# CVPR23/Depth-guided-Texture-Diffusion-for-Image-Semantic-Segmentation

Hardware: AMD Instinct MI355X
Metric: training images/sec (512x512 RGB-D, bs=8 per GPU; fwd+loss+bwd+allreduce+AdamW) (higher is better)
Workload: dtype bf16; 1 GPU; config/sod.yml model `cod` (pvt_v2_b2 + ConvNeXt-B texture diffuser + Hitnet decoder), 512x512 RGB+depth, batch 8/GPU, random init, DropPath active; mode=train, global_batch=8, parallelism=dp1, hip_graph=True, graph_mode=single

## Files before the change

### depth-guided-texture-diffusion-for-image-semantic-segmentation_amd/_lib.py

```python
from __future__ import annotations

import ctypes as C
import os

import torch

_HERE = os.path.dirname(os.path.abspath(__file__))
LIB_PATH = os.path.join(_HERE, "libdgtd.so")

F32, BF16, F64, F16 = 0, 1, 2, 3
_vp, _fp, _i, _i64, _f = C.c_void_p, C.c_void_p, C.c_int, C.c_int64, C.c_float

SIGNATURES = {
    "dgtd_version": (_i, []),
    "dgtd_last_error": (C.c_char_p, []),
    "dgtd_profile_enable": (_i, [_i]),
    "dgtd_profile_dump": (_i64, [C.c_char_p, _i64]),
    "dgtd_profile_empty": (_i, [_vp]),
    "dgtd_gemm_supported": (_i, [_i, _i, _i, _i]),
    "dgtd_gemm_bias": (_i, [_vp, _vp, _vp, _vp, _i, _i, _i, _i, _vp]),
    "dgtd_gemm_bias_gelu": (_i, [_vp, _vp, _vp, _vp, _vp, _i, _i, _i, _i, _vp]),
    "dgtd_gemm_bias_residual": (_i, [_vp, _vp, _vp, _vp, _fp, _fp, _vp, _vp, _i, _i, _i, _i64, _i, _vp]),
    "dgtd_gemm_gelu_bwd_workspace": (_i64, [_i, _i]),
    "dgtd_gemm_gelu_bwd": (_i, [_vp, _vp, _vp, _vp, _vp, C.POINTER(C.c_int), _i, _i, _i, _i, _vp]),
# ... 5 lines not shown
    "dgtd_layernorm_bwd_workspace": (_i64, [_i]),
    "dgtd_layernorm_bwd": (_i, [_vp, _vp, _fp, _fp, _fp, _vp, _fp, _fp, _vp, _i64, _i, _i, _vp]),
    "dgtd_layernorm_bwd_partial": (_i, [_vp, _vp, _fp, _fp, _fp, _vp, _vp, _vp, _i64, _i, _i, C.POINTER(C.c_int), _vp]),
    "dgtd_multi_reduce": (_i, [_vp, _i, _vp]),
    "dgtd_scale_residual_bias_bwd_partial": (_i, [_vp, _vp, _fp, _fp, _vp, _vp, _i64, _i, _i64, _i, C.POINTER(C.c_int), _vp]),
    "dgtd_gelu_bias_bwd_partial": (_i, [_vp, _vp, _vp, _vp, _i64, _i, _i, C.POINTER(C.c_int), _vp]),
    "dgtd_colsum_partial": (_i, [_vp, _vp, _i64, _i, _i, C.POINTER(C.c_int), _vp]),
    "dgtd_layernorm_bwd_add": (_i, [_vp, _vp, _fp, _fp, _fp, _vp, _vp, _fp, _fp, _vp, _i64, _i, _i, _vp]),
    "dgtd_sra_attn_fwd": (_i, [_vp, _vp, _vp, _fp, _i, _i, _i, _i, _f, _i, _vp]),
    "dgtd_sra_attn_bwd_workspace": (_i64, [_i, _i, _i]),
    "dgtd_sra_attn_bwd": (_i, [_vp, _vp, _vp, _vp, _fp, _vp, _fp, _vp, _i, _i, _i, _i, _f, _i, _vp]),
    "dgtd_dwconv_fwd": (_i, [_vp, _fp, _fp, _vp, _vp, _i, _i, _i, _i, _i, _i, _i, _vp]),
    "dgtd_dwconv_bwd_weight_workspace": (_i64, [_i, _i, _i, _i, _i]),
    "dgtd_dwconv_bwd_weight": (_i, [_vp, _vp, _fp, _i, _vp, _i, _i, _i, _i, _i, _i, _vp]),
    "dgtd_dwconv_bwd_weight_partial": (_i, [_vp, _vp, _i, _vp, _i, _i, _i, _i, _i, _i, C.POINTER(C.c_int), _vp]),
    "dgtd_dwconv_bwd_weight_batched_blocks": (_i, [_i, _i, _i, _i, _i, _i]),
    "dgtd_dwconv_bwd_weight_batched": (_i, [_vp, _vp, _i, _i, _vp, _i, _i, _i, _i, _i, _i, _vp]),
    "dgtd_dwconv_pack_batched": (_i, [_vp, _vp, _vp, _vp, _vp, _i, _i, _vp]),
    "dgtd_dwconv_pack": (_i, [_vp, _vp, _fp, _i, _i, _i, _vp]),
    "dgtd_dwconv_unpack_grads": (_i, [_fp, _vp, _vp, _i, _i, _i, _vp]),
    "dgtd_scale_residual_fwd": (_i, [_vp, _vp, _fp, _fp, _vp, _i64, _i, _i64, _i, _vp]),
    "dgtd_colsum_workspace": (_i64, [_i]),
    "dgtd_scale_residual_bwd": (_i, [_vp, _vp, _fp, _fp, _vp, _fp, _vp, _i64, _i, _i64, _i, _vp]),
    "dgtd_colsum": (_i, [_vp, _vp, _i, _vp, _i64, _i, _i, _vp]),
    "dgtd_colsum2_workspace": (_i64, [_i]),
    "dgtd_scale_residual_bias_bwd": (_i, [_vp, _vp, _fp, _fp, _vp, _fp, _vp, _i, _vp, _i64, _i, _i64, _i, _vp]),
    "dgtd_gelu_bias_bwd": (_i, [_vp, _vp, _vp, _vp, _i, _vp, _i64, _i, _i, _vp]),
    "dgtd_seg_loss_workspace": (_i64, [_i, _i]),
    "dgtd_seg_loss_fwd": (_i, [_fp, _fp, _fp, _fp, _vp, _i, _i, _i, _vp]),
    "dgtd_seg_loss_bwd": (_i, [_fp, _fp, _fp, _fp, _fp, _vp, _i, _i, _i, _vp]),
    "dgtd_ssim_workspace": (_i64, []),
    "dgtd_ssim_value": (_i, [_fp, _fp, _fp, _vp, _i, _i, _i, _vp]),
    "dgtd_diffuser_fwd": (_i, [_fp, _fp, _fp, _fp, _fp, _fp, _fp, _i, _i, _vp]),
    "dgtd_diffuser_bwd": (_i, [_fp, _fp, _fp, _fp, _fp, _fp, _fp, _fp, _fp, _fp, _fp, _i, _i, _vp]),
    "dgtd_diffuse_tail_fwd": (_i, [_fp, _fp, _fp, _fp, _fp, _i, _i, _vp]),
    "dgtd_diffuse_tail_bwd_workspace": (_i64, [_i]),
    "dgtd_diffuse_tail_bwd": (_i, [_fp, _fp, _fp, _fp, _fp, _fp, _vp, _i, _i, _vp]),
    "dgtd_adamw_flat": (_i, [_fp, _fp, _fp, _fp, _vp, _i64, _f, _f, _f, _f, _f, _f, _f, _vp]),
    "dgtd_adamw_flat_amp": (_i, [_fp, _fp, _fp, _fp, _vp, _i, _i64, _f, _f, _f, _f, _f, _f, _f, _fp, _fp, _vp]),
    "dgtd_adamw_flat_g16": (_i, [_fp, _vp, _fp, _fp, _vp, _i, _i64, _f, _f, _f, _f, _f, _f, _f, _fp, _fp, _vp]),
    "dgtd_adamw_flat_clip": (_i, [_fp, _fp, _vp, _fp, _fp, _vp, _i, _i64, _f, _f, _f, _f, _f, _f, _f, _fp, _fp, _fp, _f, _vp]),
    "dgtd_grad_norm_partial": (_i, [_vp, _i, _i64, _i, _vp, _i, _vp]),
    "dgtd_grad_clip_finalize": (_i, [_vp, _i64, _i, _f, _fp, _fp, _vp]),
    "dgtd_found_inf": (_i, [_fp, _i64, _fp, _vp]),
    "dgtd_loss_scale_update": (_i, [_fp, _f, _f, _i, _vp]),
    "dgtd_im2col": (_i, [_vp, _vp, _i, _i, _i, _i, _i64, _i64, _i64, _i64, _i, _i, _i, _i, _i, _i, _i, _vp]),
# ... 127 lines not shown
```

### depth-guided-texture-diffusion-for-image-semantic-segmentation_amd/csrc/elementwise.hip

```cpp
#include "common.h"

namespace {

constexpr int EW_MAX_BLOCKS = 512;

template <typename T>
__global__ __launch_bounds__(256) void scale_residual_fwd_kernel(const T* __restrict__ x, const T* __restrict__ y,
                                                                 const float* __restrict__ s, const float* __restrict__ gamma,
                                                                 T* __restrict__ out, int64_t rows, int C, int64_t rows_per_sample) {
  typedef typename Vec16<T>::type VT;
  constexpr int V = Vec16<T>::N;
  const int CV = C / V;
  const int64_t total = rows * CV;
  for (int64_t i = (int64_t)blockIdx.x * 256 + threadIdx.x; i < total; i += (int64_t)gridDim.x * 256) {
    const int cv = (int)(i % CV);
    const int64_t r = i / CV;
    const float sb = s ? s[r / rows_per_sample] : 1.f;
    VT xv = *reinterpret_cast<const VT*>(x + i * V);
    VT yv = *reinterpret_cast<const VT*>(y + i * V);
    VT o;
#pragma unroll
    for (int j = 0; j < V; ++j) {
      const float g = gamma ? gamma[cv * V + j] : 1.f;
      o[j] = (T)((float)xv[j] + sb * g * (float)yv[j]);
    }
    *reinterpret_cast<VT*>(out + i * V) = o;
  }
}

template <typename T, int MODE>
__global__ __launch_bounds__(256) void colsum_kernel(const T* __restrict__ g, const T* __restrict__ y, const float* __restrict__ s,
                                                     const float* __restrict__ gamma, T* __restrict__ dy, float* __restrict__ ws,
                                                     int64_t rows, int C, int64_t rows_per_sample) {
  typedef typename Vec16<T>::type VT;
  constexpr int V = Vec16<T>::N;
  extern __shared__ float red[];
  const int CV = C / V;
  const int CVB = min(CV - (int)blockIdx.y * 256, 256);
  const int RG = 256 / CVB;
  const int tid = threadIdx.x;
  const int cvl = tid % CVB, rg = tid / CVB;
  const int cv = blockIdx.y * 256 + cvl;
  float acc[V];
#pragma unroll
  for (int j = 0; j < V; ++j) acc[j] = 0.f;
  float gm[V];
#pragma unroll
  for (int j = 0; j < V; ++j) gm[j] = (MODE == 1 && gamma) ? gamma[cv * V + j] : 1.f;
  if (rg < RG) {
    for (int64_t r = (int64_t)blockIdx.x * RG + rg; r < rows; r += (int64_t)gridDim.x * RG) {
      const size_t off = (size_t)r * C + (size_t)cv * V;
      VT gv = *reinterpret_cast<const VT*>(g + off);
      if (MODE == 0) {
#pragma unroll
        for (int j = 0; j < V; ++j) acc[j] += (float)gv[j];
      } else {
        const float sb = s ? s[r / rows_per_sample] : 1.f;
        VT o;
        if (MODE == 1) {
          VT yv = *reinterpret_cast<const VT*>(y + off);
#pragma unroll
          for (int j = 0; j < V; ++j) {
            const float gg = sb * (float)gv[j];
            acc[j] += gg * (float)yv[j];
            o[j] = (T)(gg * gm[j]);
          }
        } else {
#pragma unroll
          for (int j = 0; j < V; ++j) o[j] = (T)(sb * (float)gv[j]);
        }
        *reinterpret_cast<VT*>(dy + off) = o;
      }
    }
  }
  if (MODE == 2) return;
  if (rg < RG)
#pragma unroll
    for (int j = 0; j < V; ++j) red[(rg * CVB + cvl) * V + j] = acc[j];
  __syncthreads();
  for (int i = tid; i < CVB * V; i += 256) {
    float t = 0.f;
    for (int k = 0; k < RG; ++k) t += red[k * CVB * V + i];
    ws[(size_t)blockIdx.x * C + (size_t)blockIdx.y * 256 * V + i] = t;
  }
}

constexpr int MR_MAX = 48;
struct MrTable {
  const float* ws[MR_MAX];
  float* outA[MR_MAX];
  void* outB[MR_MAX];
  void* outC[MR_MAX];
  int nblocks[MR_MAX], ncols[MR_MAX], nA[MR_MAX], dtB[MR_MAX], tr_rows[MR_MAX], tr_cols[MR_MAX];
  int first_tile[MR_MAX + 1];
  int count;
};

__device__ __forceinline__ void mr_store(void* out, int dt, int i, float v) {
  DGTD_DISPATCH(dt, ((T_*)out)[i] = (T_)v);
}

__global__ __launch_bounds__(256) void multi_reduce_kernel(MrTable t) {
  __shared__ float part[8][32];
  const int tile = blockIdx.x;
  int lo = 0, hi = t.count;
  while (hi - lo > 1) { const int mid = (lo + hi) >> 1; if (t.first_tile[mid] <= tile) lo = mid; else hi = mid; }
  const int e = lo;
// ... 15 lines not shown
    }
    for (; b < nblocks; b += 8) s0 += p[(size_t)b * rs];
  }
  part[rgp][lane] = s0 + s1;
  __syncthreads();
  if (rgp == 0 && live) {
    float v = 0.f;
#pragma unroll
    for (int k = 0; k < 8; ++k) v += part[k][lane];
    if (col < nA) t.outA[e][col] = v;
    else if (trn == 0) mr_store(t.outB[e], t.dtB[e], col - nA, v);
    else if (col - nA < trn) { const int j = col - nA, tt = j / t.tr_cols[e], c = j % t.tr_cols[e]; mr_store(t.outB[e], t.dtB[e], c * t.tr_rows[e] + tt, v); }
    else mr_store(t.outC[e], t.dtB[e], col - nA - trn, v);
  }
}

template <typename T>
int check_c(int C, const char* who) {
  constexpr int V = Vec16<T>::N;
  DGTD_REQUIRE(C % V == 0, "%s: C=%d must be a multiple of %d", who, C, V);
  return 0;
}

template <typename T, int MODE>
int colsum_launch(const void* g, const void* y, const float* s, const float* gamma, void* dy, void* out, void* ws, int64_t rows,
                  int C, int64_t rps, hipStream_t st, const char* who, int out_dt = 0, int* nblocks = nullptr) {
  if (int rc = check_c<T>(C, who)) return rc;
  constexpr int V = Vec16<T>::N;
  const int CV = C / V, ncb = (int)cdiv(CV, 256);
  const int cvb0 = std::min(CV, 256), rg = 256 / cvb0;
  int gx = (int)std::max<int64_t>(1, std::min<int64_t>(cdiv(rows, (int64_t)rg * 4), EW_MAX_BLOCKS));
  const size_t lds = (size_t)256 * V * sizeof(float);
  hipLaunchKernelGGL((colsum_kernel<T, MODE>), dim3(gx, ncb), dim3(256), lds, st, (const T*)g, (const T*)y, s, gamma, (T*)dy, (float*)ws, rows, C, rps);
  DGTD_CHECK_LAUNCH(who);
  if (nblocks) { *nblocks = gx; return 0; }
  if (MODE != 2) {
    const dgtd_reduce_entry e{(const float*)ws, gx, C, out_dt == DGTD_F32 ? (float*)out : nullptr, out_dt == DGTD_F32 ? C : 0,
                              out_dt == DGTD_F32 ? nullptr : out, out_dt, 0, 0, nullptr};
    return dgtd_multi_reduce_impl(&e, 1, st);
  }
  return 0;
}


template <typename T, int MODE>
__global__ __launch_bounds__(256) void colsum2_kernel(const T* __restrict__ g, const T* __restrict__ y, const float* __restrict__ s,
                                                      const float* __restrict__ gamma, T* __restrict__ dy, float* __restrict__ ws,
                                                      int64_t rows, int C, int64_t rows_per_sample) {
  typedef typename Vec16<T>::type VT;
  constexpr int V = Vec16<T>::N;
  extern __shared__ float red[];
  const int CV = C / V;
  const int CVB = min(CV - (int)blockIdx.y * 256, 256);
  const int RG = 256 / CVB;
// ... 116 lines not shown
  DGTD_REQUIRE(rows > 0 && C > 0 && rows_per_sample > 0 && nblocks, "scale_residual_bias_bwd_partial: bad sizes");
  DGTD_PROF(st, DGTD_HBM, (gamma ? 3.0 : 2.0) * dgtd_esize(dt) * rows * C, "dgtd_scale_residual_bias_bwd[rows=%lld,C=%d]", (long long)rows, C);
  hipStream_t h = (hipStream_t)st;
  DGTD_REQUIRE(DGTD_IS_HALF(dt) || dt == DGTD_F32, "scale_residual_bias_bwd_partial: bad dtype %d", (int)dt);
  DGTD_DISPATCH(dt, return (colsum2_launch<T_, 3>(g, y, s, gamma, dy, nullptr, nullptr, 0, workspace, rows, C, rows_per_sample, h, "scale_residual_bias_bwd", nblocks)));
}

extern "C" int dgtd_gelu_bias_bwd_partial(const void* g, const void* pre, void* dpre, void* workspace, int64_t rows, int C, dgtd_dtype dt,
                                          int* nblocks, dgtd_stream st) {
  DGTD_REQUIRE(rows > 0 && C > 0 && nblocks, "gelu_bias_bwd_partial: bad sizes");
  DGTD_PROF(st, DGTD_HBM, 3.0 * dgtd_esize(dt) * rows * C, "dgtd_gelu_bias_bwd[rows=%lld,C=%d]", (long long)rows, C);
  hipStream_t h = (hipStream_t)st;
  DGTD_REQUIRE(DGTD_IS_HALF(dt) || dt == DGTD_F32, "gelu_bias_bwd_partial: bad dtype %d", (int)dt);
  DGTD_DISPATCH(dt, return (colsum2_launch<T_, 4>(g, pre, nullptr, nullptr, dpre, nullptr, nullptr, 0, workspace, rows, C, 1, h, "gelu_bias_bwd", nblocks)));
}

extern "C" int dgtd_colsum_partial(const void* x, void* workspace, int64_t rows, int C, dgtd_dtype dt, int* nblocks, dgtd_stream st) {
  DGTD_REQUIRE(rows > 0 && C > 0 && nblocks, "colsum_partial: bad sizes");
  DGTD_PROF(st, DGTD_HBM, 1.0 * dgtd_esize(dt) * rows * C, "dgtd_colsum[rows=%lld,C=%d]", (long long)rows, C);
  DGTD_REQUIRE(DGTD_IS_HALF(dt) || dt == DGTD_F32, "colsum_partial: bad dtype %d", (int)dt);
  DGTD_DISPATCH(dt, return (colsum_launch<T_, 0>(x, nullptr, nullptr, nullptr, nullptr, nullptr, workspace, rows, C, 1, (hipStream_t)st, "colsum", 0, nblocks)));
}

extern "C" int dgtd_scale_residual_fwd(const void* x, const void* y, const float* s, const float* gamma, void* out, int64_t rows,
                                       int C, int64_t rows_per_sample, dgtd_dtype dt, dgtd_stream st) {
  DGTD_PROF(st, DGTD_HBM, 3.0 * dgtd_esize(dt) * rows * C, "dgtd_scale_residual_fwd[rows=%lld,C=%d]", (long long)rows, C);
  DGTD_REQUIRE(rows > 0 && C > 0 && rows_per_sample > 0, "scale_residual_fwd: bad sizes");
  const int V = DGTD_IS_HALF(dt) ? 8 : 4;
  DGTD_REQUIRE(C % V == 0, "scale_residual_fwd: C=%d must be a multiple of %d", C, V);
  const int grid = (int)std::min<int64_t>(cdiv(rows * (C / V), 256), 256 * 16);
  DGTD_REQUIRE(DGTD_IS_HALF(dt) || dt == DGTD_F32, "scale_residual_fwd: bad dtype %d", (int)dt);
  DGTD_DISPATCH(dt, hipLaunchKernelGGL(scale_residual_fwd_kernel<T_>, dim3(grid), dim3(256), 0, (hipStream_t)st, (const T_*)x, (const T_*)y, s, gamma, (T_*)out, rows, C,
                                       rows_per_sample));
  DGTD_CHECK_LAUNCH("scale_residual_fwd");
  return 0;
}

extern "C" int64_t dgtd_colsum_workspace(int C) { return (int64_t)EW_MAX_BLOCKS * C * sizeof(float); }

extern "C" int dgtd_scale_residual_bwd(const void* g, const void* y, const float* s, const float* gamma, void* dy, float* dgamma,
                                       void* workspace, int64_t rows, int C, int64_t rows_per_sample, dgtd_dtype dt, dgtd_stream st) {
  DGTD_PROF(st, DGTD_HBM, (gamma ? 3.0 : 2.0) * dgtd_esize(dt) * rows * C, "dgtd_scale_residual_bwd[rows=%lld,C=%d]", (long long)rows, C);
  DGTD_REQUIRE(rows > 0 && C > 0 && rows_per_sample > 0, "scale_residual_bwd: bad sizes");
  DGTD_REQUIRE((gamma == nullptr) == (dgamma == nullptr), "scale_residual_bwd: gamma and dgamma go together");
  hipStream_t h = (hipStream_t)st;
  DGTD_REQUIRE(DGTD_IS_HALF(dt) || dt == DGTD_F32, "scale_residual_bwd: bad dtype %d", (int)dt);
// ... 39 lines not shown
```

### depth-guided-texture-diffusion-for-image-semantic-segmentation_amd/csrc_torch/bindings.cpp

```cpp
#include <ATen/ATen.h>
#include <atomic>
#include <algorithm>
#include <map>
#include <set>
#include <tuple>
#include <mutex>
#include <vector>
#include <c10/hip/HIPStream.h>
#include <torch/autograd.h>
#include <torch/csrc/autograd/engine.h>
#include <torch/library.h>

#include "../../include/dgtd.h"
#include "gemm.h"

namespace {

using at::Tensor;
using torch::autograd::AutogradContext;
using torch::autograd::variable_list;

inline void* stream() { return (void*)c10::hip::getCurrentHIPStream().stream(); }
inline dgtd_dtype code(const Tensor& t) {
  if (t.scalar_type() == at::kFloat) return DGTD_F32;
// ... 41 lines not shown
inline void queue_final_flush() {
  if (g_cb_queued.exchange(true)) return;
  try {
    torch::autograd::Engine::get_default_engine().queue_callback([] { g_cb_queued.store(false); flush_deferred(); });
  } catch (...) {
    g_cb_queued.store(false);
  }
}
inline void park(const Tensor& ws, int nblocks, int ncols, float* outA, int nA, void* outB, dgtd_dtype dtB, int tr_rows = 0, int tr_cols = 0,
                 void* outC = nullptr) {
  queue_final_flush();
  std::lock_guard<std::mutex> lk(g_pending_mu);
  g_pending.push_back(PendingReduce{dgtd_reduce_entry{ws.data_ptr<float>(), nblocks, ncols, outA, nA, outB, (int32_t)dtB, tr_rows, tr_cols, outC}, ws});
}
struct PendingDw { Tensor x, du; void* dw; void* db; int32_t dw_dt; bool has_bias; int B, H, W, C, K; };
static std::vector<PendingDw> g_pending_dw;

inline void park_dw(const Tensor& x, const Tensor& du, Tensor& dw, Tensor& db, bool has_bias, int C, int K) {
  queue_final_flush();
  std::lock_guard<std::mutex> lk(g_pending_mu);
  g_pending_dw.push_back(PendingDw{x, du, dw.data_ptr(), has_bias ? db.data_ptr() : nullptr, (int32_t)code(dw), has_bias, (int)x.size(0), (int)x.size(1),
                                   (int)x.size(2), C, K});
}
constexpr int ROLE_X = 0, ROLE_DY = 8, ROLE_DW = 16, NROLE = 8;
struct Hint { int64_t group = -1; int idx = 0, count = 0; };
struct Roles { int out = -1, ga = -1, gb = -1; };
static thread_local Hint t_hint;
static thread_local Roles t_roles;
void arena_roles(int64_t out, int64_t ga, int64_t gb) { t_roles = Roles{(int)out, (int)ga, (int)gb}; }
inline int take_out_role() { const int r = t_roles.out; t_roles.out = -1; return r < NROLE ? r : -1; }
inline std::pair<int, int> take_grad_roles() {
  const std::pair<int, int> r{t_roles.ga < NROLE ? t_roles.ga : -1, t_roles.gb < NROLE ? t_roles.gb : -1};
  t_roles.ga = t_roles.gb = -1;
  return r;
}
static std::map<std::pair<int64_t, int>, Tensor> g_arenas;
static std::set<std::tuple<int64_t, int, int>> g_slot_used;
static std::map<int64_t, int> g_arena_pins;
void arena_pin(int64_t group, bool on) {
  std::lock_guard<std::mutex> lk(g_pending_mu);
  if (on) ++g_arena_pins[group];
  else if (g_arena_pins.count(group) && --g_arena_pins[group] <= 0) g_arena_pins.erase(group);
}

void arena_hint(int64_t group, int64_t idx, int64_t count) { t_hint = Hint{count > 1 ? group : -1, (int)idx, (int)count}; t_roles = Roles{}; }
void arena_release(int64_t group) {
// ... 186 lines not shown
        std::vector<int> slot;
        std::vector<void*> dws, dbs;
        bool any_b = false;
        for (size_t a = 0; a < nw; ++a) {
          const void* w = bc.second[w0 + a];
          const ConvDest& d = dest.at(w);
          dws.push_back(d.dw); dbs.push_back(d.db); any_b = any_b || d.db;
          for (size_t j : by_w[w]) {
            xs.push_back(cs[j].x.data_ptr()); dys.push_back(cs[j].dy.data_ptr());
            ms.push_back(cs[j].mask.defined() ? cs[j].mask.data_ptr() : nullptr);
            slot.push_back((int)a);
          }
        }
        const int n = (int)xs.size();
        Tensor ws = at::empty({dgtd_conv3x3_wgrad_batched_workspace(n, k.B, k.H, k.W, k.Ci, k.Co)}, cs[i].x.options().dtype(at::kByte));
        check(dgtd_conv3x3_wgrad_batched(xs.data(), dys.data(), ms.data(), slot.data(), n, dws.data(), any_b ? dbs.data() : nullptr, (int)nw, ws.data_ptr(),
                                         k.B, k.H, k.W, k.Ci, k.Co, (dgtd_dtype)k.dt, stream()), "dgtd_conv3x3_wgrad_batched");
      }
    }
  }
}

static std::atomic<int64_t> g_flushed{0};
void flush_deferred() {
  {
    std::vector<PendingConv> convs;
    std::map<const void*, ConvDest> dest;
    {
      std::lock_guard<std::mutex> lk(g_pending_mu);
      convs.swap(g_pending_conv);
      dest.swap(g_conv_dest);
      g_prelu_acc.clear();
      g_conv_flip.clear();
    }
    g_flushed += (int64_t)convs.size();
    if (!convs.empty()) flush_convs(convs, dest);
  }
  std::vector<PendingReduce> todo;
  std::vector<PendingDw> dws;
  std::vector<PendingGemm> gemms;
  {
    std::lock_guard<std::mutex> lk(g_pending_mu);
    gemms.swap(g_pending_gemm);
  }
  if (!gemms.empty()) flush_gemms(gemms);
  {
    std::lock_guard<std::mutex> lk(g_pending_mu);
    todo.swap(g_pending);
    dws.swap(g_pending_dw);
  }
  std::map<const void*, CaAcc> cas;
  {
    std::lock_guard<std::mutex> lk(g_pending_mu);
    cas.swap(g_ca_acc);
  }
  for (auto& kv : cas) {
    CaAcc& a = kv.second;
    todo.push_back(PendingReduce{dgtd_reduce_entry{a.buf.data_ptr<float>(), a.count * a.rows, 2 * a.rc, (float*)a.out1, a.rc, a.out2, (int32_t)DGTD_F32, 0, 0, nullptr}, a.buf});
  }
  g_flushed += (int64_t)(gemms.size() + todo.size() + dws.size());
  if (todo.empty() && dws.empty()) return;
  std::vector<dgtd_reduce_entry> es;
  es.reserve(todo.size() + dws.size());
  for (auto& p : todo) es.push_back(p.e);
  std::vector<Tensor> keep;
  std::vector<bool> done(dws.size(), false);
  for (size_t i = 0; i < dws.size(); ++i) {
    if (done[i]) continue;
    const PendingDw& a = dws[i];
    std::vector<size_t> grp;
    for (size_t j = i; j < dws.size(); ++j) {
      const PendingDw& b = dws[j];
      if (!done[j] && b.B == a.B && b.H == a.H && b.W == a.W && b.C == a.C && b.K == a.K && b.has_bias == a.has_bias &&
          b.x.scalar_type() == a.x.scalar_type() && b.x.device() == a.x.device()) { grp.push_back(j); done[j] = true; }
    }
    const int n = (int)grp.size(), KK = a.K * a.K;
    const int blocks = dgtd_dwconv_bwd_weight_batched_blocks(n, a.B, a.H, a.W, a.C, a.K);
    const int64_t per = (int64_t)blocks * (KK + 1) * a.C;
    Tensor ws = at::empty({(int64_t)n * per}, a.x.options().dtype(at::kFloat));
    std::vector<const void*> xs(n), dus(n);
    for (int k = 0; k < n; ++k) { xs[k] = dws[grp[k]].x.data_ptr(); dus[k] = dws[grp[k]].du.data_ptr(); }
    check(dgtd_dwconv_bwd_weight_batched(xs.data(), dus.data(), n, a.has_bias ? 1 : 0, ws.data_ptr(), a.B, a.H, a.W, a.C, a.K, code(a.x), stream()),
          "dgtd_dwconv_bwd_weight_batched");
    for (int k = 0; k < n; ++k) {
      const PendingDw& d = dws[grp[k]];
      es.push_back(dgtd_reduce_entry{ws.data_ptr<float>() + (int64_t)k * per, blocks, (int32_t)((KK + 1) * a.C), nullptr, 0, d.dw, d.dw_dt, (int32_t)KK,
                                     (int32_t)a.C, d.db});
    }
// ... 33 lines not shown
      if (st && st.get() == weight.storage().unsafeGetStorageImpl() && p.C == C && p.K == K && p.dt == weight.scalar_type() &&
          p.b == (has_bias ? bias.data_ptr() : nullptr) && p.packed.device() == weight.device())
        return p.packed;
      g_prepared_dw.erase(it);
    }
  }
  Tensor packed = at::empty({(2 * KK + 1) * C}, weight.options().dtype(at::kFloat));
  check(dgtd_dwconv_pack(weight.data_ptr(), has_bias ? bias.data_ptr() : nullptr, packed.data_ptr<float>(), (int)C, (int)K, code(weight), stream()),
        "dgtd_dwconv_pack");
  if (use) {
    std::lock_guard<std::mutex> lk(g_pending_mu);
    g_prepared_dw.emplace(weight.data_ptr(),
                          PreparedDw{c10::weak_intrusive_ptr<c10::StorageImpl>(c10::intrusive_ptr<c10::StorageImpl>::reclaim_copy(weight.storage().unsafeGetStorageImpl())),
                                     weight.data_ptr(), has_bias ? bias.data_ptr() : nullptr, packed, (int)C, (int)K, weight.scalar_type()});
  }
  return packed;
}

void set_deferred(bool on) {
  if (on) {
    std::lock_guard<std::mutex> lk(g_pending_mu);
    g_pending.clear();
    g_pending_dw.clear();
    g_pending_gemm.clear();
    g_pending_conv.clear();
    g_conv_dest.clear();
    g_conv_seen.clear();
    g_prelu_acc.clear();
    g_conv_flip.clear();
    g_ca_acc.clear();
    g_uses.clear();
    g_slot_used.clear();
  } else {
    flush_deferred();
  }
  g_defer.store(on);
  if (on) refresh_prepared();
  if (on && own_gemm_on()) refresh_transposed();
}
int64_t flushed_reductions() { return g_flushed.load(); }
int64_t pending_reductions() {
  std::lock_guard<std::mutex> lk(g_pending_mu);
  return (int64_t)(g_pending.size() + g_pending_dw.size() + g_pending_gemm.size() + g_pending_conv.size() + g_ca_acc.size());
}

struct LayerNormFn : public torch::autograd::Function<LayerNormFn> {
  static Tensor forward(AutogradContext* ctx, const Tensor& x_, const Tensor& w, const Tensor& b, double eps) {
    Tensor x = x_.contiguous();
    on_device(x);
    const int64_t C = x.size(-1), rows = x.numel() / C;
    Tensor w32 = f32(w), b32 = f32(b);
    const int out_role = take_out_role();
    Tensor y = (out_role >= 0 && hinted(t_hint, x.scalar_type())) ? arena_slot(t_hint, ROLE_X + out_role, x.sizes(), x.options()) : at::empty_like(x);
    Tensor stats = at::empty({2, rows}, x.options().dtype(at::kFloat));
    check(dgtd_layernorm_fwd(x.data_ptr(), w32.data_ptr<float>(), b32.data_ptr<float>(), y.data_ptr(), stats.data_ptr<float>(),
                             stats.data_ptr<float>() + rows, rows, (int)C, (float)eps, code(x), stream()), "dgtd_layernorm_fwd");
    ctx->save_for_backward({x, w32, stats});
    note_leaf(ctx, "leaf_w", w);
    note_leaf(ctx, "leaf_b", b);
    return y;
  }
  static variable_list backward(AutogradContext* ctx, variable_list g) {
    auto saved = ctx->get_saved_variables();
    const Tensor &x = saved[0], &w32 = saved[1], &stats = saved[2];
    const int64_t C = x.size(-1), rows = x.numel() / C;
    Tensor dy = g[0].contiguous();
// ... 245 lines not shown
                                  dy.data_ptr(), has_g ? dgamma.data_ptr<float>() : nullptr, has_g ? ws.data_ptr() : nullptr, rows, (int)C,
                                  rows / B, code(y), stream()), "dgtd_scale_residual_bwd");
    if (has_g && st_of(ctx->saved_data["g_dt"]) != at::kFloat) dgamma = dgamma.to(st_of(ctx->saved_data["g_dt"]));
    return {g, dy, undefined(), dgamma};
  }
};

Tensor colsum(const Tensor& x2, at::ScalarType out_dt, bool defer) {
  const int64_t rows = x2.size(0), C = x2.size(1);
  if (C % (16 / (int64_t)x2.element_size())) return at::sum(x2, {0}, false, at::kFloat).to(out_dt);
  Tensor out = at::empty({C}, x2.options().dtype(out_dt));
  Tensor ws = at::empty({dgtd_colsum_workspace((int)C) / 4}, x2.options().dtype(at::kFloat));
  if (defer) {
    int nb = 0;
    check(dgtd_colsum_partial(x2.data_ptr(), ws.data_ptr(), rows, (int)C, code(x2), &nb, stream()), "dgtd_colsum_partial");
    const bool f = out_dt == at::kFloat;
    park(ws, nb, (int)C, f ? out.data_ptr<float>() : nullptr, f ? (int)C : 0, f ? nullptr : out.data_ptr(), code(out));
  } else {
    check(dgtd_colsum(x2.data_ptr(), out.data_ptr(), code(out), ws.data_ptr(), rows, (int)C, code(x2), stream()), "dgtd_colsum");
  }
  return out;
}

inline bool own_gemm_on() {
  static const bool on = dgemm::env_int("DGTD_OWN_GEMM", 1) != 0;
  return on;
}
inline bool aligned16(const Tensor& t) { return ((uintptr_t)t.data_ptr() & 15) == 0; }
inline bool own_ok(at::ScalarType dt, int64_t M, int64_t N, int64_t K) {
  return own_gemm_on() && is16(dt) && M < (1ll << 31) && N < (1ll << 31) && K < (1ll << 31) &&
         dgtd_gemm_supported((int)M, (int)N, (int)K, dt == at::kHalf ? DGTD_F16 : DGTD_BF16);
}
struct PreparedWt { c10::weak_intrusive_ptr<c10::StorageImpl> wstore; const void* w; Tensor wt; int rows, cols; at::ScalarType dt; };
static std::map<const void*, PreparedWt> g_prepared_wt;
static void refresh_transposed() {
  std::map<int, std::vector<PreparedWt*>> by_dt;
  {
    std::lock_guard<std::mutex> lk(g_pending_mu);
    for (auto it = g_prepared_wt.begin(); it != g_prepared_wt.end();) {
      if (it->second.wstore.expired()) it = g_prepared_wt.erase(it);
      else { by_dt[(int)it->second.dt].push_back(&it->second); ++it; }
    }
  }
  for (auto& kv : by_dt) {
    std::vector<const void*> src;
    std::vector<void*> dst;
// ... 135 lines not shown
    Tensor out = at::empty(with_last(x, w.size(0)), x2.options());
    gemm_fwd(x2, wc, bc, out.view({-1, w.size(0)}));
    ctx->save_for_backward({x2, wc});
    const Hint hint = t_hint;
    const int xr = (hinted(hint, dt) && w.scalar_type() == dt) ? find_role(hint, ROLE_X, x2) : -1;
    ctx->saved_data["hint"] = hint_iv(xr >= 0 ? hint : Hint{}, xr);
    note_leaf(ctx, "leaf_w", w);
    if (has_b) note_leaf(ctx, "leaf_b", *b_);
    ctx->saved_data["xshape"] = x.sizes().vec();
    ctx->saved_data["w_dt"] = st_id(w);
    ctx->saved_data["b_dt"] = has_b ? st_id(*b_) : (int64_t)-1;
    ctx->saved_data["need_dx"] = x.requires_grad();
    return out;
  }
  static variable_list backward(AutogradContext* ctx, variable_list g) {
    auto saved = ctx->get_saved_variables();
    const Tensor &x2 = saved[0], &wc = saved[1];
    Tensor dy2 = as_rows(g[0], x2.scalar_type());
    Tensor dx;
    if (ctx->saved_data["need_dx"].toBool()) dx = gemm_dx(dy2, wc).view(ctx->saved_data["xshape"].toIntVector());
    const Hint hint = hint_of(ctx->saved_data["hint"]);
    const int yr = (hint.group >= 0 && deferring()) ? find_role(hint, ROLE_DY, dy2) : -1;
    Tensor dw;
    if (yr >= 0 && may_defer(ctx, "leaf_w")) {
      dw = arena_slot(hint, ROLE_DW + yr, wc.sizes(), wc.options());
      park_gemm(hint, yr, x2, dy2, dw);
    } else {
      dw = gemm_dw(dy2, x2);
      const auto w_dt = st_of(ctx->saved_data["w_dt"]);
      if (dw.scalar_type() != w_dt) dw = dw.to(w_dt);
    }
    Tensor db;
    const int64_t bk = ctx->saved_data["b_dt"].toInt();
    if (bk >= 0) db = colsum(dy2, (at::ScalarType)bk, may_defer(ctx, "leaf_b"));
    return {dx, dw, db, undefined()};
  }
};

struct LinearGeluFn : public torch::autograd::Function<LinearGeluFn> {
  static Tensor forward(AutogradContext* ctx, const Tensor& x, const Tensor& w, const Tensor& b, int64_t dt_code) {
    const auto dt = from_code(dt_code);
    Tensor x2 = as_rows(x, dt);
    Tensor wc = w.scalar_type() == dt ? w : w.to(dt);
    Tensor bc = b.scalar_type() == dt ? b.contiguous() : b.to(dt);
    const int64_t Mg = x2.size(0), Kg = x2.size(1), Ng = wc.size(0);
    const bool fused = own_ok(dt, Mg, Ng, Kg) && x2.is_contiguous() && wc.is_contiguous() && aligned16(x2) && aligned16(wc) && aligned16(bc);
    Tensor pre = fused ? at::empty({Mg, Ng}, x2.options()) : gemm_fwd(x2, wc, bc);
    const Hint hint = t_hint;
    const int out_role = take_out_role();
    const bool ar = hinted(hint, dt) && w.scalar_type() == dt;
    Tensor h = (ar && out_role >= 0) ? arena_slot(hint, ROLE_X + out_role, with_last(x, w.size(0)), pre.options())
                                     : at::empty(with_last(x, w.size(0)), pre.options());
    Tensor h2 = h.view({-1, w.size(0)});
    if (fused)
      check(dgtd_gemm_bias_gelu(x2.data_ptr(), wc.data_ptr(), bc.data_ptr(), pre.data_ptr(), h2.data_ptr(), (int)Mg, (int)Ng, (int)Kg, code(x2), stream()),
            "dgtd_gemm_bias_gelu");
    else
// ... 720 lines not shown
  m.def("linear(Tensor x, Tensor weight, Tensor? bias, int dtype_code) -> Tensor", &linear);
  m.def("linear_gelu(Tensor x, Tensor weight, Tensor bias, int dtype_code) -> Tensor", &linear_gelu);
  m.def("linear_residual(Tensor h, Tensor weight, Tensor bias, Tensor x, Tensor? s, Tensor? gamma, int dtype_code) -> Tensor", &linear_residual);
  m.def("mlp_residual(Tensor v, Tensor w1, Tensor b1, Tensor w2, Tensor b2, Tensor x, Tensor? s, Tensor? gamma, int dtype_code) -> Tensor", &mlp_residual);
  m.def("gemm_ok(int M, int N, int K, int dtype_code) -> bool", &gemm_ok);
  m.def("cab(Tensor x, Tensor w0, Tensor w1, Tensor a, Tensor cw1, Tensor cw2) -> Tensor", &cab);
  m.def("conv3x3(Tensor x, Tensor weight, Tensor? bias, bool relu) -> Tensor", &conv3x3);
  m.def("conv3x3_cl(Tensor x, Tensor weight, Tensor? bias, bool relu) -> Tensor", &conv3x3_cl);
  m.def("prelu(Tensor x, Tensor a) -> Tensor", &prelu);
  m.def("ca_gate(Tensor res, Tensor x, Tensor w1, Tensor w2) -> Tensor", &ca_gate);
  m.def("bilinear_resize(Tensor x, int oh, int ow, bool align) -> Tensor", &bilinear_resize);
  m.def("sam(Tensor xh, Tensor xl, Tensor w1, Tensor w2, Tensor v1, Tensor v2) -> Tensor", &sam);
  m.def("batch_norm(Tensor x, Tensor weight, Tensor bias, Tensor(a!) running_mean, Tensor(b!) running_var, Tensor(c!) num_batches, bool training, "
        "float momentum, float eps) -> Tensor", &batch_norm);
  m.def("set_deferred(bool on) -> ()", &set_deferred);
  m.def("flush_deferred() -> ()", &flush_deferred);
  m.def("pending_reductions() -> int", &pending_reductions);
  m.def("flushed_reductions() -> int", &flushed_reductions);
  m.def("wgrad_batched(Tensor dy, Tensor x) -> Tensor", &wgrad_batched);
  m.def("set_own_wgrad(bool on) -> ()", &set_own_wgrad);
  m.def("own_wgrad() -> bool", &own_wgrad);
  m.def("own_wgrad_calls() -> int", &own_wgrad_calls);
  m.def("own_wgrad_fallbacks() -> int", &own_wgrad_fallbacks);
  m.def("set_shared_deferral(bool on) -> ()", &set_shared_deferral);
  m.def("arena_hint(int group, int idx, int count) -> ()", &arena_hint);
  m.def("arena_roles(int out, int grad_a, int grad_b) -> ()", &arena_roles);
  m.def("arena_release(int group) -> ()", &arena_release);
  m.def("arena_bytes() -> int", &arena_bytes);
  m.def("arena_pin(int group, bool on) -> ()", &arena_pin);
}
```

### include/dgtd.h

```cpp
#ifndef DGTD_H
#define DGTD_H
#include <stdint.h>

#ifdef __cplusplus
extern "C" {
#endif

typedef enum { DGTD_F32 = 0, DGTD_BF16 = 1, DGTD_F64 = 2 , DGTD_F16 = 3 } dgtd_dtype;
typedef void* dgtd_stream;

int dgtd_version(void);
const char* dgtd_last_error(void);

int dgtd_profile_enable(int on);
int64_t dgtd_profile_dump(char* buf, int64_t cap);
int dgtd_profile_empty(dgtd_stream stream);

int dgtd_layernorm_fwd(const void* x, const float* gamma, const float* beta, void* y,
                       float* mean, float* rstd, int64_t rows, int C, float eps,
                       dgtd_dtype dt, dgtd_stream s);
int64_t dgtd_layernorm_bwd_workspace(int C);
int dgtd_layernorm_bwd(const void* dy, const void* x, const float* gamma, const float* mean,
                       const float* rstd, void* dx, float* dgamma, float* dbeta, void* workspace,
                       int64_t rows, int C, dgtd_dtype dt, dgtd_stream s);
// ... 36 lines not shown
  int32_t dtB;
  int32_t tr_rows, tr_cols;
  void* outC;
} dgtd_reduce_entry;
int dgtd_multi_reduce(const dgtd_reduce_entry* entries, int n, dgtd_stream s);

int dgtd_scale_residual_fwd(const void* x, const void* y, const float* s, const float* gamma, void* out,
                            int64_t rows, int C, int64_t rows_per_sample, dgtd_dtype dt, dgtd_stream st);
int64_t dgtd_colsum_workspace(int C);
int dgtd_scale_residual_bwd(const void* g, const void* y, const float* s, const float* gamma, void* dy,
                            float* dgamma, void* workspace, int64_t rows, int C, int64_t rows_per_sample,
                            dgtd_dtype dt, dgtd_stream st);
int64_t dgtd_colsum2_workspace(int C);
int dgtd_scale_residual_bias_bwd(const void* g, const void* y, const float* s, const float* gamma, void* dy, float* dgamma,
                                 void* dbias, dgtd_dtype bias_dt, void* workspace, int64_t rows, int C,
                                 int64_t rows_per_sample, dgtd_dtype dt, dgtd_stream st);
int dgtd_gelu_bias_bwd(const void* g, const void* pre, void* dpre, void* dbias, dgtd_dtype bias_dt, void* workspace,
                       int64_t rows, int C, dgtd_dtype dt, dgtd_stream st);
int dgtd_scale_residual_bias_bwd_partial(const void* g, const void* y, const float* s, const float* gamma, void* dy, void* workspace,
                                         int64_t rows, int C, int64_t rows_per_sample, dgtd_dtype dt, int* nblocks, dgtd_stream st);
int dgtd_gelu_bias_bwd_partial(const void* g, const void* pre, void* dpre, void* workspace, int64_t rows, int C, dgtd_dtype dt,
                               int* nblocks, dgtd_stream st);
int dgtd_colsum_partial(const void* x, void* workspace, int64_t rows, int C, dgtd_dtype dt, int* nblocks, dgtd_stream st);
int dgtd_colsum(const void* x, void* out, dgtd_dtype out_dt, void* workspace, int64_t rows, int C, dgtd_dtype dt,
                dgtd_stream st);

int dgtd_gemm_supported(int M, int N, int K, dgtd_dtype dt);
int dgtd_gemm_bias(const void* a, const void* b, const void* bias, void* d, int M, int N, int K, dgtd_dtype dt, dgtd_stream s);
int dgtd_gemm_bias_gelu(const void* a, const void* b, const void* bias, void* pre, void* h, int M, int N, int K, dgtd_dtype dt,
                        dgtd_stream s);
int dgtd_gemm_bias_residual(const void* a, const void* b, const void* bias, const void* x, const float* scale, const float* gamma,
                            void* y, void* out, int M, int N, int K, int64_t rows_per_sample, dgtd_dtype dt, dgtd_stream s);
int64_t dgtd_gemm_gelu_bwd_workspace(int M, int N);
int dgtd_gemm_gelu_bwd(const void* dy, const void* w_t, const void* pre, void* dpre, void* colsum_ws, int* nblocks, int M, int N, int K,
                       dgtd_dtype dt, dgtd_stream s);
int dgtd_transpose_batched(const void* const* src, void* const* dst, const int* rows, const int* cols, int n, dgtd_dtype dt,
                           dgtd_stream s);

int dgtd_gemm_wgrad_supported(int M, int N, int K, dgtd_dtype dt);
int64_t dgtd_gemm_wgrad_workspace(int batch, int M, int N, int K);
int dgtd_gemm_wgrad_batched(const void* dy, const void* x, void* dw, void* workspace, int batch, int M, int N, int K, int64_t s_dy,
                            int64_t s_x, int64_t s_dw, dgtd_dtype dt, dgtd_stream s);

int64_t dgtd_seg_loss_workspace(int B, int S);
int dgtd_seg_loss_fwd(const float* lo, const float* label, const float* mix, float* loss, void* workspace,
                      int B, int S, int hs, dgtd_stream s);
// ... 121 lines not shown
```

Measured before the change: 272.2 images/s.

## Defer linear bias-gradient column sums and batch them into one grouped kernel

Linear-layer bias gradients in backward are no longer reduced one at a time. They are queued and flushed together through a new grouped column-sum kernel that uses a table of pointers and a binary search over workgroup offsets. The partial results then feed the existing batched final reduction. This is meant to cut per-layer kernel launches and small under-filled grids, at the cost of holding dy tensors alive (capped at 64MB) and extra host-side bookkeeping.

```diff
diff --git a/depth-guided-texture-diffusion-for-image-semantic-segmentation_amd/_lib.py b/depth-guided-texture-diffusion-for-image-semantic-segmentation_amd/_lib.py
--- a/depth-guided-texture-diffusion-for-image-semantic-segmentation_amd/_lib.py
+++ b/depth-guided-texture-diffusion-for-image-semantic-segmentation_amd/_lib.py
@@ -51,6 +51,8 @@
     "dgtd_scale_residual_fwd": (_i, [_vp, _vp, _fp, _fp, _vp, _i64, _i, _i64, _i, _vp]),
     "dgtd_colsum_workspace": (_i64, [_i]),
     "dgtd_scale_residual_bwd": (_i, [_vp, _vp, _fp, _fp, _vp, _fp, _vp, _i64, _i, _i64, _i, _vp]),
+    "dgtd_colsum_batched_workspace": (_i64, [C.POINTER(C.c_int64), C.POINTER(C.c_int), _i, _i]),
+    "dgtd_colsum_batched": (_i, [C.POINTER(C.c_void_p), C.POINTER(C.c_int64), C.POINTER(C.c_int), _i, _i, _vp, C.POINTER(C.c_int), _vp]),
     "dgtd_colsum": (_i, [_vp, _vp, _i, _vp, _i64, _i, _i, _vp]),
     "dgtd_colsum2_workspace": (_i64, [_i]),
     "dgtd_scale_residual_bias_bwd": (_i, [_vp, _vp, _fp, _fp, _vp, _fp, _vp, _i, _vp, _i64, _i, _i64, _i, _vp]),
diff --git a/depth-guided-texture-diffusion-for-image-semantic-segmentation_amd/csrc/elementwise.hip b/depth-guided-texture-diffusion-for-image-semantic-segmentation_amd/csrc/elementwise.hip
--- a/depth-guided-texture-diffusion-for-image-semantic-segmentation_amd/csrc/elementwise.hip
+++ b/depth-guided-texture-diffusion-for-image-semantic-segmentation_amd/csrc/elementwise.hip
@@ -29,18 +29,18 @@
 }
 
 template <typename T, int MODE>
-__global__ __launch_bounds__(256) void colsum_kernel(const T* __restrict__ g, const T* __restrict__ y, const float* __restrict__ s,
-                                                     const float* __restrict__ gamma, T* __restrict__ dy, float* __restrict__ ws,
-                                                     int64_t rows, int C, int64_t rows_per_sample) {
+__device__ __forceinline__ void colsum_block(const T* __restrict__ g, const T* __restrict__ y, const float* __restrict__ s,
+                                             const float* __restrict__ gamma, T* __restrict__ dy, float* __restrict__ ws,
+                                             int64_t rows, int C, int64_t rows_per_sample, int bx, int by, int gx) {
   typedef typename Vec16<T>::type VT;
   constexpr int V = Vec16<T>::N;
   extern __shared__ float red[];
   const int CV = C / V;
-  const int CVB = min(CV - (int)blockIdx.y * 256, 256);
+  const int CVB = min(CV - by * 256, 256);
   const int RG = 256 / CVB;
   const int tid = threadIdx.x;
   const int cvl = tid % CVB, rg = tid / CVB;
-  const int cv = blockIdx.y * 256 + cvl;
+  const int cv = by * 256 + cvl;
   float acc[V];
 #pragma unroll
   for (int j = 0; j < V; ++j) acc[j] = 0.f;
@@ -48,7 +48,7 @@
 #pragma unroll
   for (int j = 0; j < V; ++j) gm[j] = (MODE == 1 && gamma) ? gamma[cv * V + j] : 1.f;
   if (rg < RG) {
-    for (int64_t r = (int64_t)blockIdx.x * RG + rg; r < rows; r += (int64_t)gridDim.x * RG) {
+    for (int64_t r = (int64_t)bx * RG + rg; r < rows; r += (int64_t)gx * RG) {
       const size_t off = (size_t)r * C + (size_t)cv * V;
       VT gv = *reinterpret_cast<const VT*>(g + off);
       if (MODE == 0) {
@@ -81,8 +81,34 @@
   for (int i = tid; i < CVB * V; i += 256) {
     float t = 0.f;
     for (int k = 0; k < RG; ++k) t += red[k * CVB * V + i];
-    ws[(size_t)blockIdx.x * C + (size_t)blockIdx.y * 256 * V + i] = t;
-  }
+    ws[(size_t)bx * C + (size_t)by * 256 * V + i] = t;
+  }
+}
+
+template <typename T, int MODE>
+__global__ __launch_bounds__(256) void colsum_kernel(const T* __restrict__ g, const T* __restrict__ y, const float* __restrict__ s,
+                                                     const float* __restrict__ gamma, T* __restrict__ dy, float* __restrict__ ws,
+                                                     int64_t rows, int C, int64_t rows_per_sample) {
+  colsum_block<T, MODE>(g, y, s, gamma, dy, ws, rows, C, rows_per_sample, (int)blockIdx.x, (int)blockIdx.y, (int)gridDim.x);
+}
+
+constexpr int CB_MAX = 64;
+struct CbTable {
+  const void* x[CB_MAX];
+  float* ws[CB_MAX];
+  int64_t rows[CB_MAX];
+  int C[CB_MAX], gx[CB_MAX];
+  int first[CB_MAX + 1];
+  int count;
+};
+
+template <typename T>
+__global__ __launch_bounds__(256) void colsum_batched_kernel(CbTable t) {
+  const int wg = blockIdx.x;
+  int lo = 0, hi = t.count;
+  while (hi - lo > 1) { const int mid = (lo + hi) >> 1; if (t.first[mid] <= wg) lo = mid; else hi = mid; }
+  const int e = lo, local = wg - t.first[e], gx = t.gx[e];
+  colsum_block<T, 0>((const T*)t.x[e], nullptr, nullptr, nullptr, nullptr, t.ws[e], t.rows[e], t.C[e], 1, local % gx, local / gx, gx);
 }
 
 constexpr int MR_MAX = 48;
@@ -144,14 +170,19 @@
   return 0;
 }
 
+struct ColsumGeom { int gx, ncb; };
+static ColsumGeom colsum_geom(int64_t rows, int C, int V) {
+  const int CV = C / V, rg = 256 / std::min(CV, 256);
+  return ColsumGeom{(int)std::max<int64_t>(1, std::min<int64_t>(cdiv(rows, (int64_t)rg * 4), EW_MAX_BLOCKS)), (int)cdiv(CV, 256)};
+}
+
 template <typename T, int MODE>
 int colsum_launch(const void* g, const void* y, const float* s, const float* gamma, void* dy, void* out, void* ws, int64_t rows,
                   int C, int64_t rps, hipStream_t st, const char* who, int out_dt = 0, int* nblocks = nullptr) {
   if (int rc = check_c<T>(C, who)) return rc;
   constexpr int V = Vec16<T>::N;
-  const int CV = C / V, ncb = (int)cdiv(CV, 256);
-  const int cvb0 = std::min(CV, 256), rg = 256 / cvb0;
-  int gx = (int)std::max<int64_t>(1, std::min<int64_t>(cdiv(rows, (int64_t)rg * 4), EW_MAX_BLOCKS));
+  const ColsumGeom geo = colsum_geom(rows, C, V);
+  const int gx = geo.gx, ncb = geo.ncb;
   const size_t lds = (size_t)256 * V * sizeof(float);
   hipLaunchKernelGGL((colsum_kernel<T, MODE>), dim3(gx, ncb), dim3(256), lds, st, (const T*)g, (const T*)y, s, gamma, (T*)dy, (float*)ws, rows, C, rps);
   DGTD_CHECK_LAUNCH(who);
@@ -314,6 +345,51 @@
   DGTD_DISPATCH(dt, return (colsum_launch<T_, 0>(x, nullptr, nullptr, nullptr, nullptr, nullptr, workspace, rows, C, 1, (hipStream_t)st, "colsum", 0, nblocks)));
 }
 
+extern "C" int64_t dgtd_colsum_batched_workspace(const int64_t* rows, const int* C, int n, dgtd_dtype dt) {
+  if (n <= 0 || !rows || !C || !(DGTD_IS_HALF(dt) || dt == DGTD_F32)) return 0;
+  const int V = 16 / dgtd_esize(dt);
+  int64_t floats = 0;
+  for (int i = 0; i < n; ++i) {
+    if (rows[i] <= 0 || C[i] <= 0 || C[i] % V) return 0;
+    floats += (int64_t)colsum_geom(rows[i], C[i], V).gx * C[i];
+  }
+  return floats * (int64_t)sizeof(float);
+}
+
+extern "C" int dgtd_colsum_batched(const void* const* x, const int64_t* rows, const int* C, int n, dgtd_dtype dt, void* workspace, int* nblocks,
+                                   dgtd_stream st) {
+  DGTD_REQUIRE(n > 0 && x && rows && C && workspace && nblocks, "colsum_batched: bad arguments");
+  DGTD_REQUIRE(DGTD_IS_HALF(dt) || dt == DGTD_F32, "colsum_batched: bad dtype %d", (int)dt);
+  const int V = 16 / dgtd_esize(dt);
+  double bytes = 0;
+  for (int i = 0; i < n; ++i) {
+    DGTD_REQUIRE(x[i] && rows[i] > 0 && C[i] > 0 && C[i] % V == 0, "colsum_batched: bad entry %d (rows=%lld, C=%d must be a multiple of %d)", i,
+                 (long long)rows[i], C[i], V);
+    bytes += 1.0 * dgtd_esize(dt) * rows[i] * C[i];
+  }
+  DGTD_PROF(st, DGTD_HBM, bytes, "dgtd_colsum_batched[n=%d]", n);
+  float* ws = (float*)workspace;
+  for (int b0 = 0; b0 < n; b0 += CB_MAX) {
+    CbTable t;
+    const int m = std::min(CB_MAX, n - b0);
+    t.count = m;
+    int wgs = 0;
+    for (int i = 0; i < m; ++i) {
+      const ColsumGeom geo = colsum_geom(rows[b0 + i], C[b0 + i], V);
+      t.x[i] = x[b0 + i]; t.ws[i] = ws; t.rows[i] = rows[b0 + i]; t.C[i] = C[b0 + i]; t.gx[i] = geo.gx; t.first[i] = wgs;
+      nblocks[b0 + i] = geo.gx;
+      ws += (size_t)geo.gx * C[b0 + i];
+      wgs += geo.gx * geo.ncb;
+    }
+    for (int i = m; i < CB_MAX; ++i) { t.x[i] = nullptr; t.ws[i] = nullptr; t.rows[i] = 0; t.C[i] = 0; t.gx[i] = 1; }
+    for (int i = m; i <= CB_MAX; ++i) t.first[i] = wgs;
+    const size_t lds = (size_t)256 * V * sizeof(float);
+    DGTD_DISPATCH(dt, hipLaunchKernelGGL(colsum_batched_kernel<T_>, dim3(wgs), dim3(256), lds, (hipStream_t)st, t));
+    DGTD_CHECK_LAUNCH("colsum_batched");
+  }
+  return 0;
+}
+
 extern "C" int dgtd_scale_residual_fwd(const void* x, const void* y, const float* s, const float* gamma, void* out, int64_t rows,
                                        int C, int64_t rows_per_sample, dgtd_dtype dt, dgtd_stream st) {
   DGTD_PROF(st, DGTD_HBM, 3.0 * dgtd_esize(dt) * rows * C, "dgtd_scale_residual_fwd[rows=%lld,C=%d]", (long long)rows, C);
diff --git a/depth-guided-texture-diffusion-for-image-semantic-segmentation_amd/csrc_torch/bindings.cpp b/depth-guided-texture-diffusion-for-image-semantic-segmentation_amd/csrc_torch/bindings.cpp
--- a/depth-guided-texture-diffusion-for-image-semantic-segmentation_amd/csrc_torch/bindings.cpp
+++ b/depth-guided-texture-diffusion-for-image-semantic-segmentation_amd/csrc_torch/bindings.cpp
@@ -87,6 +87,16 @@
   g_pending_dw.push_back(PendingDw{x, du, dw.data_ptr(), has_bias ? db.data_ptr() : nullptr, (int32_t)code(dw), has_bias, (int)x.size(0), (int)x.size(1),
                                    (int)x.size(2), C, K});
 }
+struct PendingColsum { Tensor x; void* out; int32_t out_dt; int64_t rows; int C; };
+static std::vector<PendingColsum> g_pending_colsum;
+constexpr int64_t COLSUM_HOLD_MAX = 64ll << 20;
+static int64_t g_colsum_held = 0;
+static std::atomic<int64_t> g_bias_batched{0}, g_bias_immediate{0};
+static std::atomic<bool> g_bias_force_immediate{false};
+void set_bias_colsum_immediate(bool on) { g_bias_force_immediate.store(on); }
+int64_t bias_colsum_batched() { return g_bias_batched.load(); }
+int64_t bias_colsum_immediate() { return g_bias_immediate.load(); }
+
 constexpr int ROLE_X = 0, ROLE_DY = 8, ROLE_DW = 16, NROLE = 8;
 struct Hint { int64_t group = -1; int idx = 0, count = 0; };
 struct Roles { int out = -1, ga = -1, gb = -1; };
@@ -319,6 +329,31 @@
 }
 
 static std::atomic<int64_t> g_flushed{0};
+static void flush_colsums(std::vector<PendingColsum>& cs, std::vector<dgtd_reduce_entry>& es, std::vector<Tensor>& keep) {
+  std::vector<bool> done(cs.size(), false);
+  for (size_t i = 0; i < cs.size(); ++i) {
+    if (done[i]) continue;
+    std::vector<size_t> grp;
+    for (size_t j = i; j < cs.size(); ++j)
+      if (!done[j] && cs[j].x.scalar_type() == cs[i].x.scalar_type() && cs[j].x.device() == cs[i].x.device()) { grp.push_back(j); done[j] = true; }
+    const int n = (int)grp.size();
+    std::vector<const void*> xs(n);
+    std::vector<int64_t> rows(n);
+    std::vector<int> Cs(n), nbs(n);
+    for (int k = 0; k < n; ++k) { xs[k] = cs[grp[k]].x.data_ptr(); rows[k] = cs[grp[k]].rows; Cs[k] = cs[grp[k]].C; }
+    const dgtd_dtype dt = code(cs[i].x);
+    Tensor ws = at::empty({dgtd_colsum_batched_workspace(rows.data(), Cs.data(), n, dt) / 4}, cs[i].x.options().dtype(at::kFloat));
+    check(dgtd_colsum_batched(xs.data(), rows.data(), Cs.data(), n, dt, ws.data_ptr(), nbs.data(), stream()), "dgtd_colsum_batched");
+    float* p = ws.data_ptr<float>();
+    for (int k = 0; k < n; ++k) {
+      const PendingColsum& c = cs[grp[k]];
+      const bool f = c.out_dt == (int32_t)DGTD_F32;
+      es.push_back(dgtd_reduce_entry{p, nbs[k], c.C, f ? (float*)c.out : nullptr, f ? c.C : 0, f ? nullptr : c.out, c.out_dt, 0, 0, nullptr});
+      p += (int64_t)nbs[k] * c.C;
+    }
+    keep.push_back(ws);
+  }
+}
 void flush_deferred() {
   {
     std::vector<PendingConv> convs;
@@ -336,6 +371,7 @@
   std::vector<PendingReduce> todo;
   std::vector<PendingDw> dws;
   std::vector<PendingGemm> gemms;
+  std::vector<PendingColsum> colsums;
   {
     std::lock_guard<std::mutex> lk(g_pending_mu);
     gemms.swap(g_pending_gemm);
@@ -345,6 +381,8 @@
     std::lock_guard<std::mutex> lk(g_pending_mu);
     todo.swap(g_pending);
     dws.swap(g_pending_dw);
+    colsums.swap(g_pending_colsum);
+    g_colsum_held = 0;
   }
   std::map<const void*, CaAcc> cas;
   {
@@ -355,12 +393,13 @@
     CaAcc& a = kv.second;
     todo.push_back(PendingReduce{dgtd_reduce_entry{a.buf.data_ptr<float>(), a.count * a.rows, 2 * a.rc, (float*)a.out1, a.rc, a.out2, (int32_t)DGTD_F32, 0, 0, nullptr}, a.buf});
   }
-  g_flushed += (int64_t)(gemms.size() + todo.size() + dws.size());
-  if (todo.empty() && dws.empty()) return;
+  g_flushed += (int64_t)(gemms.size() + todo.size() + dws.size() + colsums.size());
+  if (todo.empty() && dws.empty() && colsums.empty()) return;
   std::vector<dgtd_reduce_entry> es;
-  es.reserve(todo.size() + dws.size());
+  es.reserve(todo.size() + dws.size() + colsums.size());
   for (auto& p : todo) es.push_back(p.e);
   std::vector<Tensor> keep;
+  flush_colsums(colsums, es, keep);
   std::vector<bool> done(dws.size(), false);
   for (size_t i = 0; i < dws.size(); ++i) {
     if (done[i]) continue;
@@ -440,6 +479,8 @@
     std::lock_guard<std::mutex> lk(g_pending_mu);
     g_pending.clear();
     g_pending_dw.clear();
+    g_pending_colsum.clear();
+    g_colsum_held = 0;
     g_pending_gemm.clear();
     g_pending_conv.clear();
     g_conv_dest.clear();
@@ -459,7 +500,7 @@
 int64_t flushed_reductions() { return g_flushed.load(); }
 int64_t pending_reductions() {
   std::lock_guard<std::mutex> lk(g_pending_mu);
-  return (int64_t)(g_pending.size() + g_pending_dw.size() + g_pending_gemm.size() + g_pending_conv.size() + g_ca_acc.size());
+  return (int64_t)(g_pending.size() + g_pending_dw.size() + g_pending_colsum.size() + g_pending_gemm.size() + g_pending_conv.size() + g_ca_acc.size());
 }
 
 struct LayerNormFn : public torch::autograd::Function<LayerNormFn> {
@@ -751,6 +792,30 @@
   return out;
 }
 
+Tensor bias_grad(const Tensor& dy2, at::ScalarType out_dt, bool defer, bool held) {
+  const int64_t rows = dy2.size(0), C = dy2.size(1);
+  const bool chunks = C % (16 / (int64_t)dy2.element_size()) == 0;
+  if (defer && chunks && rows > 0 && !g_bias_force_immediate.load(std::memory_order_relaxed)) {
+    const int64_t bytes = held ? 0 : dy2.numel() * (int64_t)dy2.element_size();
+    bool room;
+    {
+      std::lock_guard<std::mutex> lk(g_pending_mu);
+      room = g_colsum_held + bytes <= COLSUM_HOLD_MAX;
+      if (room) g_colsum_held += bytes;
+    }
+    if (room) {
+      Tensor out = at::empty({C}, dy2.options().dtype(out_dt));
+      queue_final_flush();
+      std::lock_guard<std::mutex> lk(g_pending_mu);
+      g_pending_colsum.push_back(PendingColsum{dy2, out.data_ptr(), (int32_t)code(out), rows, (int)C});
+      ++g_bias_batched;
+      return out;
+    }
+  }
+  if (chunks) ++g_bias_immediate;
+  return colsum(dy2, out_dt, defer);
+}
+
 inline bool own_gemm_on() {
   static const bool on = dgemm::env_int("DGTD_OWN_GEMM", 1) != 0;
   return on;
@@ -932,9 +997,11 @@
     const Hint hint = hint_of(ctx->saved_data["hint"]);
     const int yr = (hint.group >= 0 && deferring()) ? find_role(hint, ROLE_DY, dy2) : -1;
     Tensor dw;
+    bool parked_w = false;
     if (yr >= 0 && may_defer(ctx, "leaf_w")) {
       dw = arena_slot(hint, ROLE_DW + yr, wc.sizes(), wc.options());
       park_gemm(hint, yr, x2, dy2, dw);
+      parked_w = true;
     } else {
       dw = gemm_dw(dy2, x2);
       const auto w_dt = st_of(ctx->saved_data["w_dt"]);
@@ -942,7 +1009,7 @@
     }
     Tensor db;
     const int64_t bk = ctx->saved_data["b_dt"].toInt();
-    if (bk >= 0) db = colsum(dy2, (at::ScalarType)bk, may_defer(ctx, "leaf_b"));
+    if (bk >= 0) db = bias_grad(dy2, (at::ScalarType)bk, may_defer(ctx, "leaf_b"), parked_w);
     return {dx, dw, db, undefined()};
   }
 };
@@ -1709,6 +1776,9 @@
   m.def("own_wgrad() -> bool", &own_wgrad);
   m.def("own_wgrad_calls() -> int", &own_wgrad_calls);
   m.def("own_wgrad_fallbacks() -> int", &own_wgrad_fallbacks);
+  m.def("set_bias_colsum_immediate(bool on) -> ()", &set_bias_colsum_immediate);
+  m.def("bias_colsum_batched() -> int", &bias_colsum_batched);
+  m.def("bias_colsum_immediate() -> int", &bias_colsum_immediate);
   m.def("set_shared_deferral(bool on) -> ()", &set_shared_deferral);
   m.def("arena_hint(int group, int idx, int count) -> ()", &arena_hint);
   m.def("arena_roles(int out, int grad_a, int grad_b) -> ()", &arena_roles);
diff --git a/include/dgtd.h b/include/dgtd.h
--- a/include/dgtd.h
+++ b/include/dgtd.h
@@ -82,6 +82,9 @@
 int dgtd_gelu_bias_bwd_partial(const void* g, const void* pre, void* dpre, void* workspace, int64_t rows, int C, dgtd_dtype dt,
                                int* nblocks, dgtd_stream st);
 int dgtd_colsum_partial(const void* x, void* workspace, int64_t rows, int C, dgtd_dtype dt, int* nblocks, dgtd_stream st);
+int64_t dgtd_colsum_batched_workspace(const int64_t* rows, const int* C, int n, dgtd_dtype dt);
+int dgtd_colsum_batched(const void* const* x, const int64_t* rows, const int* C, int n, dgtd_dtype dt, void* workspace, int* nblocks,
+                        dgtd_stream st);
 int dgtd_colsum(const void* x, void* out, dgtd_dtype out_dt, void* workspace, int64_t rows, int C, dgtd_dtype dt,
                 dgtd_stream st);
 
```

Measured after the change: 275.3 images/s, median of 6. Within noise of the previous version (+1.1%).
